# tukaani-project/xz

Hardware: AMD Instinct MI355X
Metric: compress MB/s + ratio vs xz -T0 -6, 4 GiB input, 1/2/4/8 MI355X (higher is better)
Workload: dtype u8

## Files before the change

### xz_amd/csrc/lzma_find.hip

```cpp
#include <hip/hip_runtime.h>
#include <stdint.h>
#include "kernels_api.h"
#include "kernels_internal.h"
#include "wave.h"
#include "match_common.h"

namespace {

constexpr uint32_t FIND_RUN = 256;

__device__ __forceinline__ uint32_t match16(const uint4& a, const uint4& b)
{
    const uint32_t d0 = a.x ^ b.x, d1 = a.y ^ b.y, d2 = a.z ^ b.z, d3 = a.w ^ b.w;
    const uint32_t off = d0 ? 0u : d1 ? 4u : d2 ? 8u : 12u;
    const uint32_t d = d0 ? d0 : d1 ? d1 : d2 ? d2 : d3;
    return d ? off + ((uint32_t)__builtin_ctz(d) >> 3) : 16u;
}

__device__ __forceinline__ uint32_t lane_cmplen16_from(const uint8_t* __restrict__ in, uint32_t q, uint32_t x, uint32_t len,
        uint32_t lim)
{
    while (len + 16 <= lim) {
        uint4 a, b;
        __builtin_memcpy(&a, in + q + len, 16);
        __builtin_memcpy(&b, in + x + len, 16);
        const uint32_t m = match16(a, b);
        len += m;
        if (m < 16) return len;
    }
    while (len < lim && in[q + len] == in[x + len]) ++len;
    return len;
}

__device__ __forceinline__ uint32_t prefix_max_half(uint32_t v)
{
    v = max(v, (uint32_t)__builtin_amdgcn_update_dpp(0, (int)v, 0x111, 0xF, 0xF, false));
    v = max(v, (uint32_t)__builtin_amdgcn_update_dpp(0, (int)v, 0x112, 0xF, 0xF, false));
    v = max(v, (uint32_t)__builtin_amdgcn_update_dpp(0, (int)v, 0x114, 0xF, 0xF, false));
    v = max(v, (uint32_t)__builtin_amdgcn_update_dpp(0, (int)v, 0x118, 0xF, 0xF, false));
    v = max(v, (uint32_t)__builtin_amdgcn_update_dpp(0, (int)v, 0x142, 0xA, 0xF, false));
    return v;
}

struct SnArgs {
    const uint8_t* __restrict__ in;
    const uint32_t* __restrict__ sa;
    const uint32_t* __restrict__ sa_rank;
    const uint32_t* __restrict__ prev2;
    const uint32_t* __restrict__ prev4;
    const uint32_t* __restrict__ prev8;
    const uint32_t* __restrict__ prev16;
    const uint32_t* __restrict__ prev24;
    const uint32_t* __restrict__ prev32;
    uint32_t mode;
};
constexpr uint32_t SEED_RUNS = XZAMD_SEED_LEN / 256 + 1;
constexpr uint32_t SN_WMAX = 5;

constexpr uint32_t SN_NONE = 0xFFFFFFFFu;
constexpr uint32_t ROW_RUN = FIND_RUN / 4;

template <int N>
__device__ __forceinline__ uint32_t row_ror(uint32_t v)
{
    return (uint32_t)__builtin_amdgcn_update_dpp(0, (int)v, 0x120 + N, 0xF, 0xF, false);
}
template <int N>
__device__ __forceinline__ uint32_t row_shr(uint32_t v)
{
    return (uint32_t)__builtin_amdgcn_update_dpp(0, (int)v, 0x110 + N, 0xF, 0xF, false);
}

template <int N>
__device__ __forceinline__ void pareto_step(uint32_t dist, uint32_t Lok, uint32_t t, bool& dom, uint32_t& rank)
{
    const uint32_t dj = row_ror<N>(dist), Lj = row_ror<N>(Lok), tj = row_ror<N>(t);
    const bool before = Lj != 0 && (dj < dist || (dj == dist && tj < t));
    dom = dom || (before && (Lj >= Lok || dj == dist));
    rank += before ? 1u : 0u;
}
template <int N>
__device__ __forceinline__ void count_step(uint32_t key, uint32_t t, uint32_t& idx)
{
    const uint32_t kj = row_ror<N>(key), tj = row_ror<N>(t);
    idx += (kj < key || (kj == key && tj < t)) ? 1u : 0u;
}

__global__ __launch_bounds__(64) void k_find_sn(xzamd_span_args a, SnArgs sn, uint16_t* __restrict__ mlen,
        uint32_t* __restrict__ mdist)
{
    const uint32_t lane = threadIdx.x;
    const uint32_t t = lane & 15, row = lane >> 4;
    uint32_t run = blockIdx.x;
    if (sn.mode == 1) {
        const uint32_t b = blockIdx.x / SEED_RUNS, j = blockIdx.x - b * SEED_RUNS;
        const uint32_t bs = b * a.block_size;
        run = bs / FIND_RUN + j;
        if ((uint64_t)run * FIND_RUN >= (uint64_t)bs + XZAMD_SEED_LEN || (uint64_t)run * FIND_RUN >= a.n) return;
    } else if (sn.mode == 2) {
        const uint32_t x0 = run * FIND_RUN;
        const uint32_t b = x0 / a.block_size, bs = b * a.block_size;
        const uint64_t be = (uint64_t)bs + a.block_size;
        if (x0 < bs + XZAMD_SEED_LEN || ((uint64_t)x0 + FIND_RUN > be && be < a.n)) return;
    }
    const uint32_t xr0 = run * FIND_RUN + row * ROW_RUN;
    const uint8_t* __restrict__ in = sn.in;
    const uint32_t W = a.sa_window;
    const uint32_t cyclic = a.dict_size + 1;
    const uint32_t nice = a.nice_len;
    const uint32_t n = a.n;
    const bool left = t < 5, right = t >= 5 && t < 10;
    const uint32_t k = left ? t : t - 5;
    const bool win_lane = (left || right) && k < W;
    const bool hash_lane = t >= 10;
    const uint32_t* __restrict__ hp = t == 10 ? sn.prev2 : t == 11 ? sn.prev24 : t == 12 ? sn.prev4 : t == 13 ? sn.prev8
            : t == 14 ? sn.prev16 : sn.prev32;
    const uint32_t hstride = 1u;
    const uint32_t minlen = t == 10 ? 2u : 4u;
    const bool sh1 = t != 0 && t != 5, sh2 = (left && t >= 2) || (right && t >= 7), sh4 = (left && t >= 4) || (right && t >= 9);

    uint32_t g_bs, g_be;
    {
        const uint32_t p = xr0 < n ? xr0 : 0u;
        const uint32_t blk = p / a.block_size;
        g_bs = blk * a.block_size;
        g_be = min(n, g_bs + a.block_size);
    }
    auto geo_next = [&](uint32_t& bs, uint32_t& be, uint32_t p) {
        const bool nb = p >= be;
        bs = nb ? be : bs;
        be = nb ? min(n, be + a.block_size) : be;
    };
    auto clampp = [&](uint32_t p) -> uint32_t { return p < n ? p : n - 1; };
    auto window = [&](uint32_t r, uint32_t bs, uint32_t be, bool live) -> uint32_t {
        const int32_t slot = right ? (int32_t)(r + 1 + k) : (int32_t)r - 1 - (int32_t)k;
        const bool inb = live && win_lane && slot >= (int32_t)bs && slot < (int32_t)be;
        return inb ? sn.sa[slot] : SN_NONE;
    };
    auto candidate = [&](uint32_t p, uint32_t wq, uint32_t hw, uint32_t& q, bool& valid) {
        const bool elig = wq != SN_NONE && wq < p && p - wq < cyclic;
        const uint32_t v = elig ? wq + 1 : 0u;
        uint32_t pm = v;
        { const uint32_t o = row_shr<1>(pm); pm = max(pm, sh1 ? o : 0u); }
        { const uint32_t o = row_shr<2>(pm); pm = max(pm, sh2 ? o : 0u); }
        { const uint32_t o = row_shr<4>(pm); pm = max(pm, sh4 ? o : 0u); }
        const uint32_t o1 = row_shr<1>(pm);
        const uint32_t ex = sh1 ? o1 : 0u;
        valid = elig && v > ex;
        q = elig ? wq : 0u;
        bool dup = false;
        { const uint32_t o = row_shr<1>(hw); dup = dup || (t >= 11 && o == hw); }
        { const uint32_t o = row_shr<2>(hw); dup = dup || (t >= 12 && o == hw); }
        { const uint32_t o = row_shr<3>(hw); dup = dup || (t >= 13 && o == hw); }
        { const uint32_t o = row_shr<4>(hw); dup = dup || (t >= 14 && o == hw); }
        { const uint32_t o = row_shr<5>(hw); dup = dup || (t >= 15 && o == hw); }
        if (hash_lane) {
            valid = hw != 0 && hw < cyclic && hw <= p && !dup;
            q = valid ? p - hw : 0u;
        }
    };
    auto load16 = [&](uint32_t off) -> uint4 {
        uint4 v;
        __builtin_memcpy(&v, in + off, 16);
        return v;
    };

    const uint32_t xend = min(n, xr0 + ROW_RUN);
    uint32_t g1_bs = g_bs, g1_be = g_be;
    geo_next(g1_bs, g1_be, xr0 + 1);
    uint32_t g2_bs = g1_bs, g2_be = g1_be;
    geo_next(g2_bs, g2_be, xr0 + 2);
    uint32_t rk1 = sn.sa_rank[clampp(xr0 + 1)];
    uint32_t rk2 = sn.sa_rank[clampp(xr0 + 2)];
    uint32_t hw1 = hash_lane ? hp[hstride * clampp(xr0 + 1)] : 0u;
    uint32_t w1 = window(rk1, g1_bs, g1_be, xr0 + 1 < xend);
    uint32_t q0; bool v0;
    {
        const uint32_t rk0 = sn.sa_rank[clampp(xr0)];
        const uint32_t hw0 = hash_lane ? hp[hstride * clampp(xr0)] : 0u;
        candidate(xr0, window(rk0, g_bs, g_be, xr0 < xend), hw0, q0, v0);
        if (!(xr0 < xend)) v0 = false;
    }
    bool pf0 = xr0 + 16 <= n;
    uint4 A0 = make_uint4(0, 0, 0, 0), B0 = A0;
    if (pf0) { A0 = load16(q0); B0 = load16(xr0); }

    uint32_t macc = 0;
    uint32_t i = 0;
    for (; i < ROW_RUN; ++i) {
        const uint32_t x = xr0 + i;
        if (__builtin_amdgcn_readfirstlane((int)(blockIdx.x * FIND_RUN + i)) >= (int)n) break;
        const uint32_t w2 = window(rk2, g2_bs, g2_be, x + 2 < xend);
        const uint32_t rk3 = sn.sa_rank[clampp(x + 3)];
        const uint32_t hw2 = hash_lane ? hp[hstride * clampp(x + 2)] : 0u;
        uint32_t q1; bool v1;
        candidate(x + 1, w1, hw1, q1, v1);
        if (!(x + 1 < xend)) { v1 = false; q1 = 0; }
        const bool pf1 = x + 1 + 16 <= n;
        uint4 A1 = A0, B1 = B0;
        if (pf1) { A1 = load16(q1); B1 = load16(x + 1); }
        uint32_t mval = 0;
        if (x < xend) {
            const uint32_t q = q0;
            const bool valid = v0;
            const uint32_t avail = g_be - x;
            const uint32_t buf_avail = avail < MATCH_LEN_MAX ? avail : MATCH_LEN_MAX;
            const uint32_t len_limit = nice <= avail ? nice : avail;
            const bool mf_ok = nice <= avail || avail >= 4;
            const uint64_t rec_base = (uint64_t)x * LIST_W;
            const uint32_t lim = (valid && mf_ok) ? len_limit : 0u;
            uint32_t L;
            if (pf0) {
                const uint32_t m = match16(A0, B0);
                L = m < lim ? m : lim;
                if (m == 16 && lim > 16) L = lane_cmplen16_from(in, q, x, 16, lim);
            } else {
                L = lane_cmplen16_from(in, q, x, 0, lim);
            }
            const bool ok = lim != 0 && L >= minlen;
            const uint32_t dist = x - q;
            const uint32_t Lok = ok ? L : 0u;
            bool dom = false;
            uint32_t rank = 0;
            pareto_step<1>(dist, Lok, t, dom, rank); pareto_step<2>(dist, Lok, t, dom, rank); pareto_step<3>(dist, Lok, t, dom, rank);
            pareto_step<4>(dist, Lok, t, dom, rank); pareto_step<5>(dist, Lok, t, dom, rank); pareto_step<6>(dist, Lok, t, dom, rank);
            pareto_step<7>(dist, Lok, t, dom, rank); pareto_step<8>(dist, Lok, t, dom, rank); pareto_step<9>(dist, Lok, t, dom, rank);
            pareto_step<10>(dist, Lok, t, dom, rank); pareto_step<11>(dist, Lok, t, dom, rank); pareto_step<12>(dist, Lok, t, dom, rank);
            pareto_step<13>(dist, Lok, t, dom, rank); pareto_step<14>(dist, Lok, t, dom, rank); pareto_step<15>(dist, Lok, t, dom, rank);
            const bool keep = ok && !dom;
            const uint32_t key = keep ? rank : 0xFFu;
            uint32_t kidx = 0;
            count_step<1>(key, t, kidx); count_step<2>(key, t, kidx); count_step<3>(key, t, kidx); count_step<4>(key, t, kidx);
            count_step<5>(key, t, kidx); count_step<6>(key, t, kidx); count_step<7>(key, t, kidx); count_step<8>(key, t, kidx);
            count_step<9>(key, t, kidx); count_step<10>(key, t, kidx); count_step<11>(key, t, kidx); count_step<12>(key, t, kidx);
            count_step<13>(key, t, kidx); count_step<14>(key, t, kidx); count_step<15>(key, t, kidx);
            const uint64_t kmask = __ballot(keep);
            const uint32_t cnt = (uint32_t)__builtin_popcount((uint32_t)(kmask >> (lane & 48)) & 0xFFFFu);
            const bool top = keep && kidx + 1 == cnt, second = keep && kidx + 2 == cnt;
            uint32_t len_out = L;
            if (top && L == nice) len_out = lane_cmplen16_from(in, q, x, L, buf_avail);
            uint32_t l2 = 0;
            if ((top || second) && len_out + 1 < avail) {
                const uint32_t lim2 = min(avail, len_out + 1 + LEN2_MAX);
                l2 = lane_cmplen16_from(in, q, x, len_out + 1, lim2) - (len_out + 1);
            }
            const uint32_t drop = cnt > LIST_K ? cnt - LIST_K : 0;
            if (keep && kidx >= drop) {
                const uint64_t o = rec_base + (kidx - drop);
                if (a.list_packed) {
                    mdist[o] = (len_out << 23) | (dist - 1);
                } else {
                    mlen[o] = (uint16_t)len_out;
                    mdist[o] = dist - 1;
                }
            }
            uint8_t* tr = reinterpret_cast<uint8_t*>(mdist + rec_base + LIST_K);
            if (cnt == 0) {
                if (t == 0) mdist[rec_base + LIST_K] = 0;
            } else {
                if (top) {
                    *reinterpret_cast<uint16_t*>(tr) = (uint16_t)((cnt - drop) | (l2 << 8));
                    tr[3] = 0;
                    if (cnt == 1) tr[2] = 0;
                    mval = len_out | ((dist > 1 ? 32u - (uint32_t)__builtin_clz(dist - 1) : 0u) << 9);
                }
                if (second) tr[2] = (uint8_t)l2;
            }
        }
        {
            uint32_t rv = mval;
            rv |= row_ror<1>(rv); rv |= row_ror<2>(rv); rv |= row_ror<4>(rv); rv |= row_ror<8>(rv);
            macc = t == (i & 15u) ? rv : macc;
            if ((i & 15u) == 15u) {
                const uint32_t px = xr0 + (i & ~15u) + t;
                if (px < xend) a.mtop[px] = (uint16_t)macc;
            }
        }
        q0 = q1; v0 = v1; pf0 = pf1; A0 = A1; B0 = B1;
        w1 = w2; hw1 = hw2;
        rk2 = rk3;
        g_bs = g1_bs; g_be = g1_be;
        g1_bs = g2_bs; g1_be = g2_be;
        geo_next(g2_bs, g2_be, x + 3);
    }
    if (i & 15u) {
        const uint32_t px = xr0 + (i & ~15u) + t;
        if (t < (i & 15u) && px < xend) a.mtop[px] = (uint16_t)macc;
    }
}

constexpr uint32_t EST_LONG = 4;

__global__ __launch_bounds__(256) void k_span_est(xzamd_span_args a, uint32_t nblocks, uint32_t cpb,
        uint32_t* __restrict__ est, unsigned long long* __restrict__ totals)
{
    const uint32_t t = blockIdx.x * blockDim.x + threadIdx.x;
    const uint32_t nch = nblocks * cpb;
    if (t >= nch) return;
    const uint32_t b = t / cpb, c = t - b * cpb;
    const uint32_t bs = b * a.block_size;
    const uint32_t be = min(a.n, bs + a.block_size);
    const uint64_t c0_ = (uint64_t)bs + (uint64_t)c * XZAMD_EST_CHUNK;
    uint32_t w = 0, bits = 0;
    if (c0_ < be) {
        const uint32_t c0 = (uint32_t)c0_;
        const uint32_t c1 = be - c0 < XZAMD_EST_CHUNK ? be : c0 + XZAMD_EST_CHUNK;
        uint32_t x = c0, gnext = c0;
        uint32_t cb = 0xFFFFFFFFu;
        uint4 buf = make_uint4(0, 0, 0, 0);
        while (x < c1) {
            const uint32_t base = x & ~7u;
            if (base != cb) { buf = *reinterpret_cast<const uint4*>(a.mtop + base); cb = base; }
            const uint32_t k = x & 7u;
            const uint32_t wv = k < 2 ? buf.x : k < 4 ? buf.y : k < 6 ? buf.z : buf.w;
            const uint32_t v = (k & 1u) ? wv >> 16 : wv & 0xFFFFu;
            const uint32_t len = v & 0x1FFu, bl = v >> 9;
            if (x >= gnext) {
                if (len >= 3 || (len == 2 && bl <= 7)) {
                    bits += 14 + bl;
                    gnext = x + len;
                } else {
                    bits += 6;
                    gnext = x + 1;
                }
            }
            if (len >= a.nice_len) { w += EST_LONG; x += len; }
            else { w += 1; x += 1; }
        }
        atomicAdd(&totals[b], (unsigned long long)w);
        atomicAdd(&totals[nblocks], (unsigned long long)w);
    }
    est[t] = w;
    est[nch + t] = bits;
}

__device__ __forceinline__ uint32_t wave_incl_sum(uint32_t v)
{
    const uint32_t lane = threadIdx.x;
#pragma unroll
    for (int s = 1; s < 64; s <<= 1) {
        const uint32_t o = __shfl_up(v, s);
        if (lane >= (uint32_t)s) v += o;
    }
    return v;
}

__global__ __launch_bounds__(64) void k_span_cut(xzamd_span_args a, uint32_t nblocks, uint32_t cpb,
        const uint32_t* __restrict__ est, unsigned long long* __restrict__ totals, uint32_t* __restrict__ span_tab,
        uint32_t* __restrict__ span_cnt, uint32_t cost_min, uint32_t bits_min, uint32_t min_len,
        uint32_t* __restrict__ enc_tab, uint32_t* __restrict__ enc_cnt, uint32_t* __restrict__ span_key)
{
    const uint32_t lane = threadIdx.x;
    const uint32_t b = blockIdx.x;
    const uint32_t nch = nblocks * cpb;
    const uint32_t bs = b * a.block_size;
    const uint32_t be = min(a.n, bs + a.block_size);
    const uint32_t m = (be - bs + XZAMD_EST_CHUNK - 1) / XZAMD_EST_CHUNK;
    const unsigned long long T = cost_min;
    if (b == 0 && lane == 0) totals[nblocks + 1] = T;
    const uint32_t* wk = est + (uint64_t)b * cpb;
    const uint32_t* bt = est + nch + (uint64_t)b * cpb;
    const bool two = a.enc_bits != 0;
    const uint32_t seed_chunks = two && be - bs > XZAMD_SEED_LEN ? XZAMD_SEED_LEN / XZAMD_EST_CHUNK : 0u;
    unsigned long long total = 0, total_bits = 0, all_bits = 0;
    for (uint32_t c0 = 0; c0 < m; c0 += 64) {
        const uint32_t c = c0 + lane;
        const uint32_t vb = c < m ? bt[c] : 0u, vw = c < m ? wk[c] : 0u;
        const bool planned = c >= seed_chunks;
        all_bits += lane_of(wave_incl_sum(vb), 63);
        total_bits += lane_of(wave_incl_sum(planned ? vb : 0u), 63);
        total += lane_of(wave_incl_sum(planned ? vw : 0u), 63);
    }
    unsigned long long k = total / T;
    if (bits_min) {
        const unsigned long long kb = total_bits / (unsigned long long)bits_min;
        if (kb < k) k = kb;
    }
    if (k == 0) k = 1;
    const unsigned long long Tb = (total + k - 1) / k;
    unsigned long long ke = two ? all_bits / a.enc_bits : 1ull;
    if (ke > (be - bs) / XZAMD_ENC_MIN_LEN) ke = (be - bs) / XZAMD_ENC_MIN_LEN;
    if (ke == 0) ke = 1;
    const unsigned long long Eb = (all_bits + ke - 1) / ke;
    uint32_t* tab = span_tab + 2ull * b * a.max_spb;
    uint32_t* etab = two ? enc_tab + 2ull * b * a.max_esb : nullptr;
    uint32_t ns = 1, start = 0;
    uint32_t ne = 1, estart = 0;
    unsigned long long carry_w = 0;
    unsigned long long carry_b = 0;
    if (lane == 0) { tab[0] = bs; if (two) etab[0] = bs; }
    for (uint32_t c0 = 0; c0 < m; c0 += 64) {
        const uint32_t c = c0 + lane;
        const uint32_t pw = wave_incl_sum(c < m ? wk[c] : 0u);
        const uint32_t pb = two ? wave_incl_sum(c < m ? bt[c] : 0u) : 0u;
        uint32_t subw = 0;
        uint32_t subb = 0;
        for (;;) {
            const unsigned long long accw = carry_w + (pw - subw);
            const unsigned long long len = (unsigned long long)(c + 1 - start) * XZAMD_EST_CHUNK;
            const bool cut = c + 1 < m && c >= start && ns < a.max_spb
                    && (len >= XZAMD_SPAN_MAX || (accw >= Tb && len >= min_len) || c + 1 == seed_chunks);
            const uint64_t mask = __builtin_amdgcn_ballot_w64(cut);
            if (!mask) break;
            const uint32_t L = (uint32_t)__builtin_ctzll(mask);
            start = c0 + L + 1;
            const unsigned long long closed = carry_w + (lane_of(pw, L) - subw);
            subw = lane_of(pw, L);
            carry_w = 0;
            const uint32_t p = bs + start * XZAMD_EST_CHUNK;
            if (lane == 0) {
                tab[2 * ns - 1] = p;
                tab[2 * ns] = p;
                span_key[(uint64_t)b * a.max_spb + ns - 1] = ~(uint32_t)min(closed ? closed : 1ull, 0xFFFFFFFEull);
            }
            ++ns;
            if (two) {
                const unsigned long long accb = carry_b + (lane_of(pb, L) - subb);
                if (accb >= Eb && (unsigned long long)(start - estart) * XZAMD_EST_CHUNK >= XZAMD_ENC_MIN_LEN && ne < a.max_esb) {
                    if (lane == 0) { etab[2 * ne - 1] = p; etab[2 * ne] = p; }
                    ++ne;
                    estart = start;
                    subb = lane_of(pb, L);
                    carry_b = 0;
                }
            }
        }
        carry_w += lane_of(pw, 63) - subw;
        carry_b += lane_of(pb, 63) - subb;
    }
    if (lane == 0) {
        tab[2 * ns - 1] = be;
        span_cnt[b] = ns;
        span_key[(uint64_t)b * a.max_spb + ns - 1] = ~(uint32_t)min(carry_w ? carry_w : 1ull, 0xFFFFFFFEull);
        if (two) { etab[2 * ne - 1] = be; enc_cnt[b] = ne; }
    }
}

__global__ __launch_bounds__(256) void k_part_ends(xzamd_span_args a, uint32_t nblocks, uint32_t cpb, const uint32_t* __restrict__ est,
        uint32_t* __restrict__ part_tab)
{
    const uint32_t slot = blockIdx.x * blockDim.x + threadIdx.x;
    if (slot >= nblocks * a.max_spb) return;
    const uint32_t blk = slot / a.max_spb, k = slot - blk * a.max_spb;
    if (k >= a.span_cnt[blk]) return;
    const uint32_t bs = blk * a.block_size;
    const uint32_t s0 = a.span_tab[2 * slot], pe = a.span_tab[2 * slot + 1];
    uint32_t end = pe;
    if (k != 0 && pe - s0 > XZAMD_PART_MIN) {
        const uint32_t* wk = est + (uint64_t)blk * cpb;
        const uint32_t c0 = (s0 - bs) / XZAMD_EST_CHUNK, c1 = (pe - bs + XZAMD_EST_CHUNK - 1) / XZAMD_EST_CHUNK;
        unsigned long long total = 0, acc = 0;
        for (uint32_t c = c0; c < c1; ++c) total += wk[c];
        const unsigned long long target = (total + 7) / 8;
        for (uint32_t c = c0; c < c1; ++c) {
            const uint64_t b64 = (uint64_t)bs + (uint64_t)c * XZAMD_EST_CHUNK;
            if (acc + wk[c] / 2 >= target && b64 >= (uint64_t)s0 + XZAMD_PART_MIN) { end = (uint32_t)b64; break; }
            acc += wk[c];
        }
    }
    part_tab[slot] = end;
}

__global__ __launch_bounds__(64) void k_find_exact(xzamd_span_args a, uint16_t* __restrict__ mlen,
        uint32_t* __restrict__ mdist)
{
    const uint32_t lane = threadIdx.x;
    const uint32_t x0 = blockIdx.x * FIND_RUN;
    if (x0 >= a.n) return;
    const uint32_t x1 = min(a.n, x0 + FIND_RUN);
    Env e;
    e.in = a.in; e.rank = a.rank; e.sorted_pos = a.sorted_pos; e.prev2 = a.prev2; e.prev3 = a.prev3;
    e.nice = a.nice_len; e.depth = a.depth; e.hb = a.hash_bytes; e.cyclic = a.dict_size + 1;
    e.block_end = 0; e.n_last = a.n - 1;
    e.mlen = nullptr; e.mdist = nullptr; e.packed = a.list_packed;
    Pre P;
    P.valid = false; P.pos = 0; P.ent = 0;
    P.a.rk = P.a.d2 = P.a.d3 = 0; P.an = P.a;
    uint32_t span_end = 0;
    for (uint32_t x = x0; x < x1; ++x) {
        if (x >= span_end) {
            const uint32_t blk = x / a.block_size;
            const uint32_t block_start = blk * a.block_size;
            const uint32_t block_end = min(a.n, block_start + a.block_size);
            const uint64_t k = (x - block_start) / a.span_size;
            const uint64_t se = (uint64_t)block_start + (k + 1) * a.span_size;
            span_end = se < block_end ? (uint32_t)se : block_end;
            e.block_end = block_end;
        }
        Round R;
        do_round<false>(e, P, x, span_end, 0, 0, 0, 0, R);
        const uint64_t lt = (1ull << lane) - 1;
        const bool rec = (R.mask >> lane) & 1;
        const uint32_t idx = (uint32_t)__builtin_popcountll(R.mask & lt);
        const uint32_t cnt = (uint32_t)__builtin_popcountll(R.mask);
        const uint32_t drop = cnt > LIST_K ? cnt - LIST_K : 0;
        const uint64_t rec_base = (uint64_t)x * LIST_W;
        if (rec && idx >= drop) {
            const uint32_t len = idx + 1 == cnt ? R.longest : R.L;
            const uint64_t o = rec_base + (idx - drop);
            if (e.packed) {
                mdist[o] = (len << 23) | R.D;
            } else {
                mlen[o] = (uint16_t)len;
                mdist[o] = R.D;
            }
        }
        if (lane == 0) mdist[rec_base + LIST_K] = cnt - drop;
    }
}

}

extern "C" {

int xzk_find_matches(const xzamd_span_args* a, const uint32_t* sa, const uint32_t* sa_rank, const uint32_t* prev4,
        const uint64_t* rp8, const uint64_t* rp16, const uint32_t* prev24, const uint32_t* prev32,
        uint16_t* mlen, uint32_t* mdist, int part, void* stream_)
{
    hipStream_t st = (hipStream_t)stream_;
    const uint32_t runs = (a->n + FIND_RUN - 1) / FIND_RUN;
    if (runs == 0) return 0;
    if (a->sa_window) {
        if (!sa || !sa_rank || !prev4 || !rp8 || !rp16 || !prev24 || !prev32 || !a->mtop || a->sa_window > SN_WMAX)
            return (int)hipErrorInvalidValue;
        if (part != 0 && a->block_size < XZAMD_SEED_LEN + 2 * FIND_RUN) return (int)hipErrorInvalidValue;
        SnArgs sn;
        sn.in = a->in; sn.sa = sa; sn.sa_rank = sa_rank; sn.prev2 = a->prev2; sn.prev4 = prev4;
        sn.prev8 = reinterpret_cast<const uint32_t*>(rp8) + a->n;
        sn.prev16 = reinterpret_cast<const uint32_t*>(rp16) + a->n;
        sn.prev24 = prev24; sn.prev32 = prev32;
        sn.mode = (uint32_t)part;
        const uint32_t nblocks = (a->n + a->block_size - 1) / a->block_size;
        hipLaunchKernelGGL(k_find_sn, dim3(part == 1 ? nblocks * SEED_RUNS : runs), dim3(64), 0, st, *a, sn, mlen, mdist);
    } else {
        hipLaunchKernelGGL(k_find_exact, dim3(runs), dim3(64), 0, st, *a, mlen, mdist);
    }
    return (int)hipGetLastError();
}

int xzk_span_plan(const xzamd_span_args* a, uint32_t nblocks, uint32_t* est, unsigned long long* totals,
        uint32_t* span_tab, uint32_t* span_cnt, uint32_t cost_min, uint32_t bits_min, uint32_t min_len,
        uint32_t* enc_tab, uint32_t* enc_cnt,
        uint32_t* order_bufs, void* sort_tmp, uint64_t sort_tmp_bytes, uint32_t** order_out, void* stream_)
{
    hipStream_t st = (hipStream_t)stream_;
    if (order_out) *order_out = nullptr;
    if (nblocks == 0 || a->n == 0) return 0;
    if (!a->mtop || a->max_spb == 0 || cost_min == 0 || !order_bufs || !order_out) return (int)hipErrorInvalidValue;
    if (a->enc_bits && (!enc_tab || !enc_cnt || a->max_esb == 0 || min_len < XZAMD_SEED_LEN)) return (int)hipErrorInvalidValue;
    const uint32_t cpb = (a->block_size + XZAMD_EST_CHUNK - 1) / XZAMD_EST_CHUNK;
    const uint32_t nslots = nblocks * a->max_spb;
    uint32_t* key_a = order_bufs;
    uint32_t* key_b = order_bufs + nslots;
    uint32_t* val_a = order_bufs + 2ull * nslots;
    uint32_t* val_b = order_bufs + 3ull * nslots;
    hipError_t e = hipMemsetAsync(totals, 0, (size_t)(nblocks + 2) * sizeof(unsigned long long), st);
    if (e == hipSuccess) e = hipMemsetAsync(key_a, 0xFF, (size_t)nslots * 4, st);
    if (e != hipSuccess) return (int)e;
    const uint64_t nch = (uint64_t)nblocks * cpb;
    hipLaunchKernelGGL(k_span_est, dim3((uint32_t)((nch + 255) / 256)), dim3(256), 0, st, *a, nblocks, cpb, est, totals);
    hipLaunchKernelGGL(k_span_cut, dim3(nblocks), dim3(64), 0, st, *a, nblocks, cpb, est, totals, span_tab, span_cnt,
            cost_min, bits_min, min_len, enc_tab, enc_cnt, key_a);
    if (a->part_tab) {
        xzamd_span_args a2 = *a;
        a2.span_tab = span_tab; a2.span_cnt = span_cnt;
        hipLaunchKernelGGL(k_part_ends, dim3((nslots + 255) / 256), dim3(256), 0, st, a2, nblocks, cpb, est, a->part_tab);
    }
    e = sort_launch_order(key_a, key_b, val_a, val_b, nslots, sort_tmp, (size_t)sort_tmp_bytes, order_out, st);
    if (e != hipSuccess) return (int)e;
    return (int)hipGetLastError();
}

}
```

Baseline: 642.3.

## Replace O(n^2) DPP pareto ranking with bitonic row sort and prefix-max filter

New measurement: 650.0, median of 6. 1.2% higher.

```diff
diff --git a/xz_amd/csrc/lzma_find.hip b/xz_amd/csrc/lzma_find.hip
--- a/xz_amd/csrc/lzma_find.hip
+++ b/xz_amd/csrc/lzma_find.hip
@@ -71,21 +71,45 @@
     return (uint32_t)__builtin_amdgcn_update_dpp(0, (int)v, 0x110 + N, 0xF, 0xF, false);
 }
 
-template <int N>
-__device__ __forceinline__ void pareto_step(uint32_t dist, uint32_t Lok, uint32_t t, bool& dom, uint32_t& rank)
-{
-    const uint32_t dj = row_ror<N>(dist), Lj = row_ror<N>(Lok), tj = row_ror<N>(t);
-    const bool before = Lj != 0 && (dj < dist || (dj == dist && tj < t));
-    dom = dom || (before && (Lj >= Lok || dj == dist));
-    rank += before ? 1u : 0u;
-}
-template <int N>
-__device__ __forceinline__ void count_step(uint32_t key, uint32_t t, uint32_t& idx)
-{
-    const uint32_t kj = row_ror<N>(key), tj = row_ror<N>(t);
-    idx += (kj < key || (kj == key && tj < t)) ? 1u : 0u;
-}
-
+constexpr uint32_t SORT_NONE = 0xFFFFFE00u;
+constexpr int DPP_XOR1 = 0xB1, DPP_XOR2 = 0x4E, DPP_XOR3 = 0x1B, DPP_XOR7 = 0x141, DPP_XOR15 = 0x140;
+constexpr int DPP_XOR4 = -1;
+
+template <int CTRL>
+__device__ __forceinline__ uint32_t row_partner(uint32_t v)
+{
+    if constexpr (CTRL == DPP_XOR4) {
+        const int up = __builtin_amdgcn_update_dpp(0, (int)v, 0x104, 0xF, 0x5, false);
+        return (uint32_t)__builtin_amdgcn_update_dpp(up, (int)v, 0x114, 0xF, 0xA, false);
+    } else {
+        return (uint32_t)__builtin_amdgcn_update_dpp(0, (int)v, CTRL, 0xF, 0xF, false);
+    }
+}
+template <bool PACKED, int CTRL>
+__device__ __forceinline__ void sort_layer(uint32_t& key, uint32_t& len, bool low)
+{
+    const uint32_t pk = row_partner<CTRL>(key);
+    if constexpr (PACKED) {
+        key = low ? min(key, pk) : max(key, pk);
+    } else {
+        const uint32_t pl = row_partner<CTRL>(len);
+        const bool take = (pk < key) != !low;
+        key = take ? pk : key;
+        len = take ? pl : len;
+    }
+}
+template <bool PACKED>
+__device__ __forceinline__ void row_sort16(uint32_t& key, uint32_t& len, bool low1, bool low2, bool low4, bool low8)
+{
+    sort_layer<PACKED, DPP_XOR1>(key, len, low1);
+    sort_layer<PACKED, DPP_XOR3>(key, len, low2);  sort_layer<PACKED, DPP_XOR1>(key, len, low1);
+    sort_layer<PACKED, DPP_XOR7>(key, len, low4);  sort_layer<PACKED, DPP_XOR2>(key, len, low2);
+    sort_layer<PACKED, DPP_XOR1>(key, len, low1);
+    sort_layer<PACKED, DPP_XOR15>(key, len, low8); sort_layer<PACKED, DPP_XOR4>(key, len, low4);
+    sort_layer<PACKED, DPP_XOR2>(key, len, low2);  sort_layer<PACKED, DPP_XOR1>(key, len, low1);
+}
+
+template <bool PACKED>
 __global__ __launch_bounds__(64) void k_find_sn(xzamd_span_args a, SnArgs sn, uint16_t* __restrict__ mlen,
         uint32_t* __restrict__ mdist)
 {
@@ -115,8 +139,9 @@
     const bool hash_lane = t >= 10;
     const uint32_t* __restrict__ hp = t == 10 ? sn.prev2 : t == 11 ? sn.prev24 : t == 12 ? sn.prev4 : t == 13 ? sn.prev8
             : t == 14 ? sn.prev16 : sn.prev32;
-    const uint32_t hstride = 1u;
     const uint32_t minlen = t == 10 ? 2u : 4u;
+    const bool low1 = !(t & 1), low2 = !(t & 2), low4 = !(t & 4), low8 = !(t & 8);
+    const uint32_t below = (1u << t) - 1;
     const bool sh1 = t != 0 && t != 5, sh2 = (left && t >= 2) || (right && t >= 7), sh4 = (left && t >= 4) || (right && t >= 9);
 
     uint32_t g_bs, g_be;
@@ -172,12 +197,12 @@
     geo_next(g2_bs, g2_be, xr0 + 2);
     uint32_t rk1 = sn.sa_rank[clampp(xr0 + 1)];
     uint32_t rk2 = sn.sa_rank[clampp(xr0 + 2)];
-    uint32_t hw1 = hash_lane ? hp[hstride * clampp(xr0 + 1)] : 0u;
+    uint32_t hw1 = hash_lane ? hp[clampp(xr0 + 1)] : 0u;
     uint32_t w1 = window(rk1, g1_bs, g1_be, xr0 + 1 < xend);
     uint32_t q0; bool v0;
     {
         const uint32_t rk0 = sn.sa_rank[clampp(xr0)];
-        const uint32_t hw0 = hash_lane ? hp[hstride * clampp(xr0)] : 0u;
+        const uint32_t hw0 = hash_lane ? hp[clampp(xr0)] : 0u;
         candidate(xr0, window(rk0, g_bs, g_be, xr0 < xend), hw0, q0, v0);
         if (!(xr0 < xend)) v0 = false;
     }
@@ -192,7 +217,7 @@
         if (__builtin_amdgcn_readfirstlane((int)(blockIdx.x * FIND_RUN + i)) >= (int)n) break;
         const uint32_t w2 = window(rk2, g2_bs, g2_be, x + 2 < xend);
         const uint32_t rk3 = sn.sa_rank[clampp(x + 3)];
-        const uint32_t hw2 = hash_lane ? hp[hstride * clampp(x + 2)] : 0u;
+        const uint32_t hw2 = hash_lane ? hp[clampp(x + 2)] : 0u;
         uint32_t q1; bool v1;
         candidate(x + 1, w1, hw1, q1, v1);
         if (!(x + 1 < xend)) { v1 = false; q1 = 0; }
@@ -201,7 +226,6 @@
         if (pf1) { A1 = load16(q1); B1 = load16(x + 1); }
         uint32_t mval = 0;
         if (x < xend) {
-            const uint32_t q = q0;
             const bool valid = v0;
             const uint32_t avail = g_be - x;
             const uint32_t buf_avail = avail < MATCH_LEN_MAX ? avail : MATCH_LEN_MAX;
@@ -213,29 +237,30 @@
             if (pf0) {
                 const uint32_t m = match16(A0, B0);
                 L = m < lim ? m : lim;
-                if (m == 16 && lim > 16) L = lane_cmplen16_from(in, q, x, 16, lim);
+                if (m == 16 && lim > 16) L = lane_cmplen16_from(in, q0, x, 16, lim);
             } else {
-                L = lane_cmplen16_from(in, q, x, 0, lim);
+                L = lane_cmplen16_from(in, q0, x, 0, lim);
             }
             const bool ok = lim != 0 && L >= minlen;
-            const uint32_t dist = x - q;
-            const uint32_t Lok = ok ? L : 0u;
-            bool dom = false;
-            uint32_t rank = 0;
-            pareto_step<1>(dist, Lok, t, dom, rank); pareto_step<2>(dist, Lok, t, dom, rank); pareto_step<3>(dist, Lok, t, dom, rank);
-            pareto_step<4>(dist, Lok, t, dom, rank); pareto_step<5>(dist, Lok, t, dom, rank); pareto_step<6>(dist, Lok, t, dom, rank);
-            pareto_step<7>(dist, Lok, t, dom, rank); pareto_step<8>(dist, Lok, t, dom, rank); pareto_step<9>(dist, Lok, t, dom, rank);
-            pareto_step<10>(dist, Lok, t, dom, rank); pareto_step<11>(dist, Lok, t, dom, rank); pareto_step<12>(dist, Lok, t, dom, rank);
-            pareto_step<13>(dist, Lok, t, dom, rank); pareto_step<14>(dist, Lok, t, dom, rank); pareto_step<15>(dist, Lok, t, dom, rank);
-            const bool keep = ok && !dom;
-            const uint32_t key = keep ? rank : 0xFFu;
-            uint32_t kidx = 0;
-            count_step<1>(key, t, kidx); count_step<2>(key, t, kidx); count_step<3>(key, t, kidx); count_step<4>(key, t, kidx);
-            count_step<5>(key, t, kidx); count_step<6>(key, t, kidx); count_step<7>(key, t, kidx); count_step<8>(key, t, kidx);
-            count_step<9>(key, t, kidx); count_step<10>(key, t, kidx); count_step<11>(key, t, kidx); count_step<12>(key, t, kidx);
-            count_step<13>(key, t, kidx); count_step<14>(key, t, kidx); count_step<15>(key, t, kidx);
-            const uint64_t kmask = __ballot(keep);
-            const uint32_t cnt = (uint32_t)__builtin_popcount((uint32_t)(kmask >> (lane & 48)) & 0xFFFFu);
+            uint32_t skey, slen;
+            if constexpr (PACKED) {
+                skey = ok ? ((x - q0 - 1) << 9) | L : SORT_NONE;
+                slen = 0;
+            } else {
+                skey = ok ? x - q0 - 1 : SN_NONE;
+                slen = ok ? L : 0u;
+            }
+            row_sort16<PACKED>(skey, slen, low1, low2, low4, low8);
+            if constexpr (PACKED) slen = skey & 0x1FFu;
+            L = slen;
+            const uint32_t dist = (PACKED ? skey >> 9 : skey) + 1;
+            const uint32_t q = x - dist;
+            uint32_t pm = L;
+            pm = max(pm, row_shr<1>(pm)); pm = max(pm, row_shr<2>(pm)); pm = max(pm, row_shr<4>(pm)); pm = max(pm, row_shr<8>(pm));
+            const bool keep = L > row_shr<1>(pm);
+            const uint32_t kept = (uint32_t)(__ballot(keep) >> (lane & 48)) & 0xFFFFu;
+            const uint32_t cnt = (uint32_t)__builtin_popcount(kept);
+            const uint32_t kidx = (uint32_t)__builtin_popcount(kept & below);
             const bool top = keep && kidx + 1 == cnt, second = keep && kidx + 2 == cnt;
             uint32_t len_out = L;
             if (top && L == nice) len_out = lane_cmplen16_from(in, q, x, L, buf_avail);
@@ -247,7 +272,7 @@
             const uint32_t drop = cnt > LIST_K ? cnt - LIST_K : 0;
             if (keep && kidx >= drop) {
                 const uint64_t o = rec_base + (kidx - drop);
-                if (a.list_packed) {
+                if constexpr (PACKED) {
                     mdist[o] = (len_out << 23) | (dist - 1);
                 } else {
                     mlen[o] = (uint16_t)len_out;
@@ -531,7 +556,9 @@
         sn.prev24 = prev24; sn.prev32 = prev32;
         sn.mode = (uint32_t)part;
         const uint32_t nblocks = (a->n + a->block_size - 1) / a->block_size;
-        hipLaunchKernelGGL(k_find_sn, dim3(part == 1 ? nblocks * SEED_RUNS : runs), dim3(64), 0, st, *a, sn, mlen, mdist);
+        const dim3 grid(part == 1 ? nblocks * SEED_RUNS : runs);
+        if (a->list_packed) hipLaunchKernelGGL(k_find_sn<true>, grid, dim3(64), 0, st, *a, sn, mlen, mdist);
+        else hipLaunchKernelGGL(k_find_sn<false>, grid, dim3(64), 0, st, *a, sn, mlen, mdist);
     } else {
         hipLaunchKernelGGL(k_find_exact, dim3(runs), dim3(64), 0, st, *a, mlen, mdist);
     }
```
